# NazirNayal8/RbA

Measured on AMD Instinct MI355X. Metric: images/sec @1024x2048 Swin-B-1dl (RbA inference hot path), higher is better.
Workload: dtype f32 (f16x3 split-MFMA GEMMs, fp32 accumulate)

## Files before the change

### include/rba_hip.h

```cpp
#ifndef RBA_HIP_H
#define RBA_HIP_H

#include <stdint.h>

#ifdef __cplusplus
extern "C" {
#endif

int rba_hip_version(void);

int rba_set_concurrent_streams(int n);

int rba_reduce_f32(const float* mask, const float* cls_prob, float* rba, float* sem_seg, int32_t* argmax,
                   int Q, int K, int64_t HW, int score_mode, void* stream);

int rba_reduce_ws_f32(const float* mask, const float* cls_prob, float* rba, float* sem_seg, int32_t* argmax, int Q, int K,
                      int64_t HW, int score_mode, void* workspace, void* stream);

int rba_reduce_up4_f32(const float* mask_lowres, const float* cls_prob, float* rba, float* sem_seg,
                       int32_t* argmax, int Q, int K, int h, int w, int crop_h, int crop_w, int score_mode, void* stream);

int rba_resample_bilinear_f32(const float* in, const float* add, float* out, int C, int h, int w, int H, int W,
                              void* stream);

// ... 40 lines not shown
int64_t rba_group_norm_nhwc_workspace_bytes(int B, int P, int C, int G);
int rba_group_norm_nhwc_f32(const float* x, const float* gamma, const float* beta, float* y, float* workspace, int B, int P, int C,
                            int G, float eps, int relu, void* stream);
int rba_resample_bilinear_nhwc_f32(const float* in, const float* add, float* out, int C, int h, int w, int H, int W, void* stream);

int rba_add_layer_norm_f32(const float* x, const float* t, const float* t_bias, const float* gamma, const float* beta,
                           float* sum_out, float* y, int64_t rows, int C, float eps, void* stream);

int rba_merge_layer_norm_f32(const float* x, const float* gamma, const float* beta, float* y, int B, int H, int W, int Cin, float eps,
                             void* stream);

int rba_skinny_linear_f32(const float* x, const float* weight, const float* bias, float* out, int M, int N, int K,
                          int relu, void* stream);
int rba_skinny_linear_add_f32(const float* x, const float* x_add, int add_cols, const float* weight, const float* bias, float* out,
                              int M, int N, int K, int relu, int seg_n, void* stream);

int rba_split_weight_bf16x3(const float* weight, void* packed, int N, int K, void* stream);
int rba_split_linear_f32(const float* x, const void* weight_packed, const float* bias, float* out, int64_t M, int N, int K,
                         int act, void* stream);

int rba_split_weight_f16x2(const float* weight, void* packed, int N, int K, void* stream);
int rba_split_linear_f16x3_f32(const float* x, const void* weight_packed, const float* bias, float* out, int64_t M, int N, int K,
                               int act, void* stream);
int rba_split_linear_f16x3_res_f32(const float* x, const void* weight_packed, const float* bias, const float* residual, float* out,
                                   int64_t M, int N, int K, void* stream);

int rba_add_layer_norm_frag_f32(const float* x, const float* t, const float* t_bias, const float* gamma, const float* beta,
                                float* sum_out, void* y_frag, int64_t rows, int C, float eps, void* stream);
int rba_split_linear_f16x3_frag_f32(const void* x_frag, const void* weight_packed, const float* bias, const float* residual, float* out,
                                    int64_t M, int N, int K, int act, void* stream);
int rba_swin_window_attn_split_out_f32(const float* qkv, const float* qkv_bias, const float* bias_frag, void* out_frag, int B, int H, int W,
                                       int nH, int hd, int ws, int shift, void* stream);
int rba_swin_attn_block_supported(int C, int ws);
int64_t rba_swin_attn_block_weight_bytes(int C);
int rba_swin_attn_block_pack_f32(const float* qkv_weight, const float* proj_weight, void* image, int C, void* stream);
int rba_swin_attn_block_f32(float* x, float* y2, const float* norm1_weight, const float* norm1_bias, float eps1, const void* weight_image,
                            const float* qkv_bias, const float* bias_frag, const float* proj_bias, const float* norm2_weight,
                            const float* norm2_bias, float eps2, int B, int H, int W, int C, int ws, int shift, void* stream);
int rba_swin_attn_qkv_supported(int C, int ws);
int rba_swin_attn_qkv_split_out_f32(const float* x, void* out_frag, const float* norm1_weight, const float* norm1_bias, float eps1,
                                    const void* weight_image, const float* qkv_bias, const float* bias_frag, int B, int H, int W, int C, int ws,
                                    int shift, void* stream);
int rba_resample_bilinear_nhwc_split_out_f32(const float* in, const float* add, void* out_frag, int C, int h, int w, int H, int W,
                                             int64_t row0, void* stream);

int rba_resample_bilinear_nhwc_gn_f32(const float* in, const float* in_mr, const float* in_gamma, const float* in_beta, int in_relu,
                                      const float* add, const float* add_mr, const float* add_gamma, const float* add_beta, void* out,
                                      int split_out, int C, int G, int h, int w, int H, int W, int64_t row0, void* stream);
int rba_group_norm_nhwc_stats_f32(const float* x, float* mr, float* workspace, int B, int P, int C, int G, float eps, void* stream);
int rba_conv3x3_nhwc_f16x3_split_in_f32(const void* x_frag, const void* weight_packed, const float* bias, float* out, int B, int H, int W,
                                        int C, int N, void* stream);
int rba_swin_mlp_fused_f16x3_f32(const float* x, const void* w1_packed, const float* b1, const void* w2_packed, const float* b2,
                                 const float* residual, float* out, int64_t M, int C, int HID, void* stream);
int rba_swin_mlp_fused_ln_f16x3_f32(float* x, const float* norm_weight, const float* norm_bias, float eps, const void* w1_packed, const float* b1,
                                    const void* w2_packed, const float* b2, int64_t M, int C, int HID, void* stream);
int rba_split_linear_f16x3_gelu_split_out(const void* x, int x_is_split, const void* weight_packed, const float* bias, void* out_frag,
                                          int64_t M, int N, int K, void* stream);

int rba_split_linear_nchw_out_f32(const float* x, const void* weight_packed, const float* bias, float* out, int64_t M, int N,
                                  int K, int rows_per_image, void* stream);

int rba_split_linear_nchw_out_f16x3_f32(const float* x, const void* weight_packed, const float* bias, float* out, int64_t M, int N, int K,
                                        int rows_per_image, void* stream);

int rba_split_linear_nchw_out_gn_f16x3_f32(const float* x, const float* mr, const float* gamma, const float* beta, int G, int relu,
                                           const void* weight_packed, const float* bias, float* out, int64_t M, int N, int K,
                                           int rows_per_image, void* stream);

int rba_conv3x3_nhwc_f32(const float* x, const void* weight_packed, const float* bias, float* out, int B, int H, int W, int C,
                         int N, void* stream);

int rba_conv3x3_nhwc_f16x3_f32(const float* x, const void* weight_packed, const float* bias, float* out, int B, int H, int W, int C,
                               int N, void* stream);

int rba_split_linear_f16x3_gn_moments_f32(const float* x, const void* weight_packed, const float* bias, float* out, int64_t M, int N, int K,
                                          int rows_per_image, int G, float* moments, void* stream);
int rba_conv3x3_nhwc_f16x3_split_in_gn_moments_f32(const void* x_frag, const void* weight_packed, const float* bias, float* out, int B, int H,
                                                   int W, int C, int N, int G, float* moments, void* stream);
int rba_group_norm_nhwc_merge_f32(const float* moments, float* mr, int B, int G, int splits, float eps, void* stream);

int rba_patch_im2col_u8(const uint8_t* image, float* out, int h, int w, int Hp, int Wp, const float* mean, const float* std, void* stream);
int rba_patch_im2col_f32(const float* image, float* out, int h, int w, int Hp, int Wp, const float* mean, const float* std, void* stream);

int rba_gaussian_blur_f32(const float* in, float* out, int H, int W, int kernel_size, float sigma, void* stream);

int rba_quad_mean_f32(const float* v, float* out, int64_t rows, int S, void* stream);
int rba_softmax_drop_last_f32(const float* logits, float* prob, int64_t rows, int K1, void* stream);

int rba_threshold_u8(const float* score, uint8_t* out, int64_t n, float threshold, void* stream);
int rba_morph3x3_u8(const uint8_t* in, uint8_t* out, int H, int W, int dilate, void* stream);
int rba_ccl4_roots_i32(const uint8_t* mask, int32_t* roots, int H, int W, void* stream);

int rba_bn_relu_conv1x1_f32(const float* x, const float* scale, const float* shift, const float* weight, const float* bias, float* out,
                            int B, int C, int O, int64_t P, void* stream);
int rba_resample_bilinear_ac_f32(const float* x, float* out, int C, int h, int w, int H, int W, void* stream);

typedef struct {
  const float* x_add;
  const void* packed;
  const float* bias;
  float* out;
  int N;
  int ld_out;
  int act;
} rba_token_linear_problem;
int rba_token_linear_pack_f16x2(const float* weight, void* packed, int N, int K, void* stream);
int rba_token_linear_f32(const float* x, const float* x_add, const void* packed, const float* bias, const float* residual,
                         const float* ln_weight, const float* ln_bias, float ln_eps, float* out, int64_t M, int N, int K, int act,
                         void* stream);
int rba_token_linear_multi_f32(const float* x, const rba_token_linear_problem* problems, int n_problems, int64_t M, int K, void* stream);

#ifdef __cplusplus
}
#endif
#endif
```

### rba_amd/_lib.py

```python
import ctypes
import os

_HERE = os.path.dirname(os.path.abspath(__file__))
LIB_PATH = os.environ.get("RBA_HIP_LIB") or os.path.join(_HERE, "csrc", "librba_hip.so")
KNOBS_LIB_PATH = os.path.join(_HERE, "csrc", "librba_hip_knobs.so")

_c_f32p = ctypes.c_void_p
_i = ctypes.c_int
_i64 = ctypes.c_int64
_vp = ctypes.c_void_p

SIGNATURES = {
    "rba_hip_version": [],
    "rba_set_concurrent_streams": [_i],
    "rba_reduce_f32": [_vp, _vp, _vp, _vp, _vp, _i, _i, _i64, _i, _vp],
    "rba_reduce_ws_f32": [_vp, _vp, _vp, _vp, _vp, _i, _i, _i64, _i, _vp, _vp],
    "rba_reduce_up4_f32": [_vp, _vp, _vp, _vp, _vp, _i, _i, _i, _i, _i, _i, _i, _vp],
    "rba_resample_bilinear_f32": [_vp, _vp, _vp, _i, _i, _i, _i, _i, _vp],
    "rba_ms_deform_attn_fwd_f32": [_vp, _vp, _vp, _vp, _vp, _vp, _i, _i, _i, _i, _i, _i, _i, _vp],
    "rba_ms_deform_attn_fwd_f64": [_vp, _vp, _vp, _vp, _vp, _vp, _i, _i, _i, _i, _i, _i, _i, _vp],
    "rba_ms_deform_attn_bwd_f32": [_vp, _vp, _vp, _vp, _vp, _vp, _vp, _vp, _vp, _i, _i, _i, _i, _i, _i, _i, _vp],
    "rba_ms_deform_attn_bwd_f64": [_vp, _vp, _vp, _vp, _vp, _vp, _vp, _vp, _vp, _i, _i, _i, _i, _i, _i, _i, _vp],
    "rba_msda_prepare_f32": [_vp, _vp, _vp, _vp, _vp, _i64, _i, _i, _i, _vp],
    "rba_resample_bilinear_nhwc_gn_f32": [_vp, _vp, _vp, _vp, _i, _vp, _vp, _vp, _vp, _vp, _i, _i, _i, _i, _i, _i, _i, _i64, _vp],
    "rba_group_norm_nhwc_stats_f32": [_vp, _vp, _vp, _i, _i, _i, _i, ctypes.c_float, _vp],
    "rba_msda_fused_f32": [_vp, _vp, _vp, _vp, _vp, _vp, _i, _i, _i, _i, _i, _i, _i, _vp],
    "rba_masked_xattn_workspace_bytes": [_i, _i, _i, _i],
    "rba_masked_xattn_f32": [_vp, _vp, _vp, _vp, _vp, _vp, _i, _i, _i, _i, _i, _vp],
    "rba_mask_logits_f32": [_vp, _vp, _vp, _i, _i, _i, _i64, _vp],
    "rba_mask_logits_f16x3_f32": [_vp, _vp, _vp, _i, _i, _i, _i64, _vp],
    "rba_swin_window_attn_f32": [_vp, _vp, _vp, _vp, _vp, _i, _i, _i, _i, _i, _i, _i, _vp],
    "rba_swin_window_attn_split_out_f32": [_vp, _vp, _vp, _vp, _i, _i, _i, _i, _i, _i, _i, _vp],
    "rba_swin_bias_fragments_elems": [_i, _i],
    "rba_swin_attn_block_supported": [_i, _i],
    "rba_swin_attn_block_weight_bytes": [_i],
    "rba_swin_attn_qkv_supported": [_i, _i],
    "rba_swin_attn_qkv_split_out_f32": [_vp, _vp, _vp, _vp, ctypes.c_float, _vp, _vp, _vp, _i, _i, _i, _i, _i, _i, _vp],
    "rba_swin_attn_block_pack_f32": [_vp, _vp, _vp, _i, _vp],
    "rba_swin_attn_block_f32": [_vp, _vp, _vp, _vp, ctypes.c_float, _vp, _vp, _vp, _vp, _vp, _vp, ctypes.c_float, _i, _i, _i, _i, _i, _i, _vp],
    "rba_swin_bias_fragments_f32": [_vp, _vp, _i, _i, _vp],
    "rba_skinny_linear_f32": [_vp, _vp, _vp, _vp, _i, _i, _i, _i, _vp],
    "rba_skinny_linear_add_f32": [_vp, _vp, _i, _vp, _vp, _vp, _i, _i, _i, _i, _i, _vp],
    "rba_split_weight_bf16x3": [_vp, _vp, _i, _i, _vp],
    "rba_split_linear_f32": [_vp, _vp, _vp, _vp, _i64, _i, _i, _i, _vp],
    "rba_split_weight_f16x2": [_vp, _vp, _i, _i, _vp],
    "rba_split_linear_f16x3_f32": [_vp, _vp, _vp, _vp, _i64, _i, _i, _i, _vp],
    "rba_split_linear_f16x3_res_f32": [_vp, _vp, _vp, _vp, _vp, _i64, _i, _i, _vp],
    "rba_split_linear_f16x3_frag_f32": [_vp, _vp, _vp, _vp, _vp, _i64, _i, _i, _i, _vp],
    "rba_swin_mlp_fused_f16x3_f32": [_vp, _vp, _vp, _vp, _vp, _vp, _vp, _i64, _i, _i, _vp],
    "rba_swin_mlp_fused_ln_f16x3_f32": [_vp, _vp, _vp, ctypes.c_float, _vp, _vp, _vp, _vp, _i64, _i, _i, _vp],
    "rba_split_linear_f16x3_gelu_split_out": [_vp, _i, _vp, _vp, _vp, _i64, _i, _i, _vp],
    "rba_split_linear_nchw_out_f32": [_vp, _vp, _vp, _vp, _i64, _i, _i, _i, _vp],
    "rba_split_linear_nchw_out_f16x3_f32": [_vp, _vp, _vp, _vp, _i64, _i, _i, _i, _vp],
    "rba_split_linear_f16x3_gn_moments_f32": [_vp, _vp, _vp, _vp, _i64, _i, _i, _i, _i, _vp, _vp],
    "rba_conv3x3_nhwc_f16x3_split_in_gn_moments_f32": [_vp, _vp, _vp, _vp, _i, _i, _i, _i, _i, _i, _vp, _vp],
    "rba_group_norm_nhwc_merge_f32": [_vp, _vp, _i, _i, _i, ctypes.c_float, _vp],
    "rba_split_linear_nchw_out_gn_f16x3_f32": [_vp, _vp, _vp, _vp, _i, _i, _vp, _vp, _vp, _i64, _i, _i, _i, _vp],
    "rba_conv3x3_nhwc_f32": [_vp, _vp, _vp, _vp, _i, _i, _i, _i, _i, _vp],
    "rba_conv3x3_nhwc_f16x3_f32": [_vp, _vp, _vp, _vp, _i, _i, _i, _i, _i, _vp],
    "rba_conv3x3_nhwc_f16x3_split_in_f32": [_vp, _vp, _vp, _vp, _i, _i, _i, _i, _i, _vp],
    "rba_resample_bilinear_nhwc_split_out_f32": [_vp, _vp, _vp, _i, _i, _i, _i, _i, _i64, _vp],
    "rba_patch_im2col_u8": [_vp, _vp, _i, _i, _i, _i, _vp, _vp, _vp],
    "rba_patch_im2col_f32": [_vp, _vp, _i, _i, _i, _i, _vp, _vp, _vp],
    "rba_group_norm_nhwc_workspace_bytes": [_i, _i, _i, _i],
    "rba_group_norm_nhwc_f32": [_vp, _vp, _vp, _vp, _vp, _i, _i, _i, _i, ctypes.c_float, _i, _vp],
    "rba_resample_bilinear_nhwc_f32": [_vp, _vp, _vp, _i, _i, _i, _i, _i, _vp],
    "rba_bn_relu_conv1x1_f32": [_vp, _vp, _vp, _vp, _vp, _vp, _i, _i, _i, _i64, _vp],
    "rba_resample_bilinear_ac_f32": [_vp, _vp, _i, _i, _i, _i, _i, _vp],
    "rba_gaussian_blur_f32": [_vp, _vp, _i, _i, _i, ctypes.c_float, _vp],
    "rba_quad_mean_f32": [_vp, _vp, _i64, _i, _vp],
    "rba_softmax_drop_last_f32": [_vp, _vp, _i64, _i, _vp],
    "rba_threshold_u8": [_vp, _vp, _i64, ctypes.c_float, _vp],
    "rba_morph3x3_u8": [_vp, _vp, _i, _i, _i, _vp],
    "rba_ccl4_roots_i32": [_vp, _vp, _i, _i, _vp],
    "rba_add_layer_norm_f32": [_vp, _vp, _vp, _vp, _vp, _vp, _vp, _i64, _i, ctypes.c_float, _vp],
    "rba_add_layer_norm_frag_f32": [_vp, _vp, _vp, _vp, _vp, _vp, _vp, _i64, _i, ctypes.c_float, _vp],
    "rba_merge_layer_norm_f32": [_vp, _vp, _vp, _vp, _i, _i, _i, _i, ctypes.c_float, _vp],
    "rba_group_norm_workspace_bytes": [_i, _i, _i, _i],
    "rba_group_norm_f32": [_vp, _vp, _vp, _vp, _vp, _i, _i, _i, _i, ctypes.c_float, _i, _vp],
    "rba_token_linear_pack_f16x2": [_vp, _vp, _i, _i, _vp],
    "rba_token_linear_f32": [_vp, _vp, _vp, _vp, _vp, _vp, _vp, ctypes.c_float, _vp, _i64, _i, _i, _i, _vp],
    "rba_token_linear_multi_f32": [_vp, _vp, _i, _i64, _i, _vp],
}

class TokenLinearProblem(ctypes.Structure):
    _fields_ = [("x_add", ctypes.c_void_p), ("packed", ctypes.c_void_p), ("bias", ctypes.c_void_p), ("out", ctypes.c_void_p),
                ("N", ctypes.c_int), ("ld_out", ctypes.c_int), ("act", ctypes.c_int)]


EXPECTED_ABI = 191

_lib = None


class RbaHipError(RuntimeError):
    pass


def load():
    global _lib
    if _lib is not None:
        return _lib
    _lib = _open(LIB_PATH)
    return _lib


_handles = {}


def _open(path):
    if path in _handles:
        return _handles[path]
    import torch
    if not os.path.exists(path):
        raise RbaHipError(
            f"{path} not found: build it with `python -m rba_amd.csrc.build` (hipcc --offload-arch=gfx950; --knobs for the knobs build). "
            "rba_amd has no CPU or PyTorch fallback for its HIP kernels.")
    lib = ctypes.CDLL(path)
    for name, argtypes in SIGNATURES.items():
        try:
            fn = getattr(lib, name)
        except AttributeError as e:
            raise RbaHipError(f"{path} does not export {name}; rebuild it") from e
        fn.argtypes = argtypes
        fn.restype = ctypes.c_int64 if name.endswith(("_bytes", "_elems")) else ctypes.c_int
    abi = int(lib.rba_hip_version())
    if abi != EXPECTED_ABI:
        raise RbaHipError(f"{path} has ABI version {abi}, these bindings are written for {EXPECTED_ABI}; rebuild it "
                          "(python -m rba_amd.csrc.build)")
    _handles[path] = lib
    return lib


class use_library:

    def __init__(self, path):
        self.path = path

    def __enter__(self):
        global _lib
        self.prev = _lib
        _lib = _open(self.path)
        return _lib

    def __exit__(self, *exc):
        global _lib
# ... 26 lines not shown
```

### rba_amd/csrc/build.py

```python
import os
import subprocess
import sys
from concurrent.futures import ThreadPoolExecutor

HERE = os.path.dirname(os.path.abspath(__file__))
SOURCES = ["rba_reduce.hip", "resample.hip", "ms_deform_attn.hip", "ms_deform_attn_bwd.hip", "masked_xattn.hip", "mask_logits.hip",
           "swin_window_attn.hip", "swin_attn_block.hip", "group_norm.hip", "layer_norm.hip", "skinny_linear.hip", "split_linear.hip", "split_linear_dma.hip", "split_linear_gnf.hip", "gaussian_blur.hip", "open_panoptic.hip", "dense_hybrid.hip", "patch_embed.hip", "token_linear.hip", "decoder_small.hip"]
HEADERS = ["common.h", "knobs.h", "rba_reduce_kernels.h", "split_linear_dma.h", "split_linear_h3.h", "split_linear_h3q.h", "mlp_fused_h3.h", "swin_window_attn_h3.h", "swin_attn_block.h",
           os.path.join("..", "..", "include", "rba_hip.h")]
TUNE_SOURCES = [os.path.join("tune", "rba_reduce_tune.hip"), os.path.join("tune", "split_linear_tune.hip"), os.path.join("tune", "split_linear_ws.hip"), os.path.join("tune", "mlp_fused_h1.hip"), os.path.join("tune", "k5_timing.hip"), os.path.join("tune", "k5_wpe_ab.hip"), os.path.join("tune", "k5_wpe_plain.hip"), os.path.join("tune", "k5_persist.hip"), os.path.join("tune", "k7_timing.hip")] + [os.path.join("tune", f"gnf_form{f}_dbg{d}.hip") for f in (0, 1) for d in (0, 1)] + [os.path.join("tune", "gnf_form0_dbg1_unpacked.hip"), os.path.join("tune", "gnf_form1_dbg0_unpacked.hip")]
TUNE_LIB = os.path.join(HERE, "tune", "librba_tune.so")
LIB = os.path.join(HERE, "librba_hip.so")
KNOBS_LIB = os.path.join(HERE, "librba_hip_knobs.so")
KNOBS = ["-DRBA_TUNE_KNOBS"]
OBJ = os.path.join(HERE, "build")
HIPCC = os.environ.get("HIPCC", "/opt/rocm/bin/hipcc")
FLAGS = ["--offload-arch=gfx950", "-O3", "-std=c++17", "-fPIC", "-ffp-contract=fast", "-Wno-unused-result"]
NO_PACKED_FP32 = ["-Xclang", "-target-feature", "-Xclang", "-packed-fp32-ops"]
MFMA_SOURCES = ({"split_linear.hip", "split_linear_dma.hip", "mask_logits.hip", "masked_xattn.hip", "skinny_linear.hip"}
                if os.environ.get("RBA_NO_PACKED_FP32") == "1" else set())
UNPACKED_ALWAYS = {"split_linear_gnf.hip", "ms_deform_attn_bwd.hip"}
UNPACKED_SOURCES = MFMA_SOURCES | UNPACKED_ALWAYS


def _run(cmd):
    r = subprocess.run(cmd, cwd=HERE, stderr=subprocess.PIPE, text=True)
    err = "\n".join(ln for ln in r.stderr.splitlines() if "not a recognized feature for this target" not in ln)
    if err.strip():
        print(err, file=sys.stderr, flush=True)
    if r.returncode:
        raise subprocess.CalledProcessError(r.returncode, cmd)


def _stale(target, deps) -> bool:
    if not os.path.exists(target):
        return True
    t = os.path.getmtime(target)
    return any(os.path.getmtime(d) > t for d in deps)


def stale() -> bool:
    return _stale(LIB, [os.path.join(HERE, f) for f in SOURCES + HEADERS])


def build(force: bool = False, verbose: bool = True, knobs: bool = False) -> str:
    lib = KNOBS_LIB if knobs else LIB
    if not force and not _stale(lib, [os.path.join(HERE, f) for f in SOURCES + HEADERS]):
        return lib
    obj_dir = os.path.join(OBJ, "knobs") if knobs else OBJ
    os.makedirs(obj_dir, exist_ok=True)
    hdrs = [os.path.join(HERE, h) for h in HEADERS]

    def compile_one(src):
        s, o = os.path.join(HERE, src), os.path.join(obj_dir, src.replace(".hip", ".o"))
        if force or _stale(o, [s] + hdrs):
            cmd = [HIPCC] + FLAGS + (KNOBS if knobs else []) + (NO_PACKED_FP32 if src in UNPACKED_SOURCES else []) + ["-c", s, "-o", o]
            if verbose:
                print(" ".join(cmd), flush=True)
            _run(cmd)
        return o

    with ThreadPoolExecutor(max_workers=min(8, os.cpu_count() or 1)) as ex:
        objs = list(ex.map(compile_one, SOURCES))
    _link_and_gate(objs, lib, verbose)
    return lib


def _link_and_gate(objs, lib, verbose):
    tmp = lib + ".unscanned"
    cmd = [HIPCC, "--offload-arch=gfx950", "-shared", "-fPIC"] + objs + ["-o", tmp]
    if verbose:
        print(" ".join(cmd), flush=True)
    subprocess.run(cmd, check=True, cwd=HERE)
    try:
        from . import isa_hazards
    except ImportError:
        sys.path.insert(0, HERE)
        import isa_hazards
    try:
        r = isa_hazards.gate(tmp)
    except Exception:
        os.remove(tmp)
        raise
    if verbose:
        print(f"isa_hazards: {os.path.basename(lib)}: {r['code_objects']} code objects clean (rules D, T, P)", flush=True)
    os.replace(tmp, lib)


def build_knobs(force: bool = False, verbose: bool = True) -> str:
    return build(force=force, verbose=verbose, knobs=True)
# ... 29 lines not shown
```

### rba_amd/modeling/backbone/swin.py

```python
from types import SimpleNamespace

import torch
import torch.nn as nn
import torch.nn.functional as F

from ... import ops
from ...lru import derived
from ...registry import BACKBONE_REGISTRY


def relative_position_index(ws: int) -> torch.Tensor:
    ar = torch.arange(ws)
    gy, gx = torch.meshgrid(ar, ar, indexing="ij")
    gy, gx = gy.reshape(-1), gx.reshape(-1)
    dy = gy[:, None] - gy[None, :] + (ws - 1)
    dx = gx[:, None] - gx[None, :] + (ws - 1)
    return dy * (2 * ws - 1) + dx


class WindowAttention(nn.Module):
    def __init__(self, dim, window_size, num_heads):
        super().__init__()
        self.dim, self.window_size, self.num_heads = dim, window_size, num_heads
        self.relative_position_bias_table = nn.Parameter(torch.zeros((2 * window_size - 1) ** 2, num_heads))
# ... 61 lines not shown
            x = ops.linear(y, a.proj, residual=x)
            hidden = self.mlp.fc1.out_features
            y = ops.add_layer_norm(x, self.norm2.weight, self.norm2.bias, self.norm2.eps, frag=ops.linear_takes_split(M, hidden, C))[1]
            y = ops.linear(y, self.mlp.fc1, gelu=True, split_out=ops.linear_takes_split(M, C, hidden))
            return ops.linear(y, self.mlp.fc2, residual=x), None
        x, y = ops.add_layer_norm(x, self.norm1.weight, self.norm1.bias, self.norm1.eps, t, tb, inplace_sum=True,
                                  frag=ops.linear_takes_split(M, 3 * C, C))
        qkv = ops.linear(y, a.qkv)
        bias, bias_frag = a.gathered_bias()
        fused = ops.linear_residual_fused(M, C, C)
        y = ops.swin_window_attn(qkv, a.qkv.bias, bias, H, W, self.num_heads, self.window_size, self.shift_size, bias_frag=bias_frag,
                                 split_out=fused and bias_frag is not None and ops.linear_takes_split(M, C, C) and
                                 ops.swin_window_attn_split_ok(C // self.num_heads, self.window_size))
        if fused:
            x = ops.linear(y, a.proj, residual=x)
            hidden = self.mlp.fc1.out_features
            if ops.mlp_fused_ok(M, C, hidden):
                y = ops.add_layer_norm(x, self.norm2.weight, self.norm2.bias, self.norm2.eps)[1]
                return ops.mlp_fused(y, self.mlp.fc1, self.mlp.fc2, x), None
            y = ops.add_layer_norm(x, self.norm2.weight, self.norm2.bias, self.norm2.eps, frag=ops.linear_takes_split(M, hidden, C))[1]
            y = ops.linear(y, self.mlp.fc1, gelu=True, split_out=ops.linear_takes_split(M, C, hidden))
            return ops.linear(y, self.mlp.fc2, residual=x), None
        t = ops.linear(y, a.proj, use_bias=False)
        x, y = ops.add_layer_norm(x, self.norm2.weight, self.norm2.bias, self.norm2.eps, t, a.proj.bias, inplace_sum=True)
        y = ops.linear(y, self.mlp.fc1, gelu=True)
        return x, (ops.linear(y, self.mlp.fc2, use_bias=False), self.mlp.fc2.bias)


class PatchMerging(nn.Module):
    def __init__(self, dim):
        super().__init__()
        self.reduction = nn.Linear(4 * dim, 2 * dim, bias=False)
        self.norm = nn.LayerNorm(4 * dim)

    def forward(self, x, H, W):
        x = ops.merge_layer_norm(x.contiguous(), H, W, self.norm.weight, self.norm.bias, self.norm.eps)
        return ops.linear(x, self.reduction)


class BasicLayer(nn.Module):
    def __init__(self, dim, depth, num_heads, window_size, mlp_ratio, downsample):
        super().__init__()
        self.blocks = nn.ModuleList(
            SwinTransformerBlock(dim, num_heads, window_size, 0 if i % 2 == 0 else window_size // 2, mlp_ratio)
            for i in range(depth))
        self.downsample = PatchMerging(dim) if downsample else None


class PatchEmbed(nn.Module):
    def __init__(self, patch_size, in_chans, embed_dim):
        super().__init__()
        self.patch_size = patch_size
        self.proj = nn.Conv2d(in_chans, embed_dim, kernel_size=patch_size, stride=patch_size)
        self.norm = nn.LayerNorm(embed_dim)

    def forward(self, x):
        ps = self.patch_size
        _, _, H, W = x.shape
        if W % ps or H % ps:
            x = F.pad(x, (0, (ps - W % ps) % ps, 0, (ps - H % ps) % ps))
        B, Cin, H, W = x.shape
        Wh, Ww = H // ps, W // ps
        cols = x.reshape(B, Cin, Wh, ps, Ww, ps).permute(0, 2, 4, 1, 3, 5).reshape(B, Wh * Ww, Cin * ps * ps).contiguous()
        x = ops.linear(cols, self._linear_view())
        return ops.add_layer_norm(x, self.norm.weight, self.norm.bias, self.norm.eps)[1], Wh, Ww

    def _linear_view(self):
        w, b = self.proj.weight, self.proj.bias
        return derived(self, "linear_view", (w, b), lambda: SimpleNamespace(weight=w.detach().reshape(w.shape[0], -1), bias=b))

    def fused_ok(self):
        w = self.proj.weight
        return self.patch_size == 4 and w.shape[1] == 3 and w.is_cuda and w.dtype == torch.float32 and ops.SPLIT_MODE == "f16x3"

    def forward_images(self, images, mean, std, Hp, Wp):
        w = self.proj.weight

        def build():
            w64 = torch.zeros((w.shape[0], 64), dtype=torch.float32, device=w.device)
            w64[:, :48] = w.detach().reshape(w.shape[0], 48)
            return ops.split_weight(w64, mode="f16x3")

        planes = derived(self, "planes64", (w,), build)
        cols = torch.stack([ops.patch_im2col(im, mean, std, Hp, Wp) for im in images]) if len(images) > 1 \
            else ops.patch_im2col(images[0], mean, std, Hp, Wp)[None]
        x = ops.split_linear(cols, planes, self.proj.bias, out_features=w.shape[0])
        return ops.add_layer_norm(x, self.norm.weight, self.norm.bias, self.norm.eps)[1], Hp // 4, Wp // 4


@BACKBONE_REGISTRY.register()
class D2SwinTransformer(nn.Module):

    def __init__(self, arch):
        super().__init__()
        E, depths = arch["embed_dim"], arch["depths"]
        self.patch_embed = PatchEmbed(arch["patch_size"], 3, E)
        self.layers = nn.ModuleList(
            BasicLayer(E * 2 ** i, depths[i], arch["num_heads"][i], arch["window_size"], arch["mlp_ratio"],
                       downsample=i < len(depths) - 1) for i in range(len(depths)))
        self.num_features = [E * 2 ** i for i in range(len(depths))]
        for i, c in enumerate(self.num_features):
            self.add_module(f"norm{i}", nn.LayerNorm(c))

    @property
    def size_divisibility(self):
        return 32

    def forward_images(self, images, mean, std, Hp, Wp):
        return self._stages(*self.patch_embed.forward_images(images, mean, std, Hp, Wp))

    def forward(self, x):
        if x.dim() != 4:
            raise ValueError(f"SwinTransformer takes an input of shape (N, C, H, W). Got {tuple(x.shape)} instead!")
        return self._stages(*self.patch_embed(x))

    def _stages(self, x, Wh, Ww):
        outs = {}
        for i, layer in enumerate(self.layers):
            pending = None
            for blk in layer.blocks:
                x, pending = blk(x, Wh, Ww, pending)
            norm = getattr(self, f"norm{i}")
            t, tb = pending if pending is not None else (None, None)
            x, y = ops.add_layer_norm(x, norm.weight, norm.bias, norm.eps, t, tb, inplace_sum=True)
            outs[f"res{i + 2}"] = y.view(-1, Wh, Ww, self.num_features[i]).permute(0, 3, 1, 2)
            if layer.downsample is not None:
                x = layer.downsample(x, Wh, Ww)
                Wh, Ww = (Wh + 1) // 2, (Ww + 1) // 2
        return outs
```

### rba_amd/ops.py

```python
import contextlib
import ctypes
import threading
import functools
import math
import os

import torch

from . import _lib
from ._lib import RbaHipError
from .lru import derived


def _stream():
    return torch.cuda.current_stream().cuda_stream


def _cuda_tensors(args):
    for a in args:
        if isinstance(a, torch.Tensor):
            if a.is_cuda:
                yield a
        elif isinstance(a, (list, tuple)):
            yield from _cuda_tensors(a)
# ... 993 lines not shown

@_hip_op
def token_linear(x, lin, x_add=None, use_bias=True, relu=False, residual=None, norm=None):
    lib = _lib.load()
    _chk(x, "x")
    N, K = lin.weight.shape
    if x.shape[-1] != K or not token_linear_ok(N, K):
        raise RbaHipError("token_linear: x [..., K] with K % 32 == 0, N <= 256 and the f16x3 mode (see token_linear_ok)")
    M = x.numel() // K
    if x_add is not None:
        _chk(x_add, "x_add")
        if tuple(x_add.shape) != tuple(x.shape):
            raise RbaHipError("x_add must have x's shape")
    bias = lin.bias if use_bias else None
    if bias is not None:
        _chk(bias, "bias", dim=1)
    out = torch.empty(tuple(x.shape[:-1]) + (N,), dtype=torch.float32, device=x.device)
    if (residual is None) != (norm is None):
        raise RbaHipError("token_linear: residual and norm come together")
    if norm is not None:
        _chk(residual, "residual")
        if tuple(residual.shape) != tuple(out.shape) or N % 16 or relu or norm.weight.numel() != N:
            raise RbaHipError("token_linear(norm=...): residual [..., N], N % 16 == 0, no activation")
        _lib.check(lib.rba_token_linear_f32(_p(x), _p(x_add), _p(_token_planes(lin)), _p(bias), _p(residual), _p(norm.weight), _p(norm.bias),
                                            float(norm.eps), _p(out), M, N, K, 0, _stream()), "rba_token_linear_f32")
        return out
    _lib.check(lib.rba_token_linear_f32(_p(x), _p(x_add), _p(_token_planes(lin)), _p(bias), None, None, None, 0.0, _p(out), M, N, K,
                                        2 if relu else 0, _stream()), "rba_token_linear_f32")
    return out


@_hip_op
def token_linear_multi(x, specs):
    lib = _lib.load()
    _chk(x, "x")
    K = x.shape[-1]
    M = x.numel() // K if K else 0
    if not 1 <= len(specs) <= 3:
        raise RbaHipError("token_linear_multi: one to three problems")
    arr = (_lib.TokenLinearProblem * len(specs))()
    outs, keep = [], []
    for i, (lin, x_add, out, col0, relu) in enumerate(specs):
        N, K_ = lin.weight.shape
        if K_ != K or not token_linear_ok(N, K) or N % 4:
            raise RbaHipError("token_linear_multi: weights [N <= 256, N % 4 == 0, K] with x's K % 32 == 0 (see token_linear_ok)")
        if x_add is not None:
            _chk(x_add, "x_add")
            if tuple(x_add.shape) != tuple(x.shape):
                raise RbaHipError("x_add must have x's shape")
        if out is None:
            out, col0 = torch.empty(tuple(x.shape[:-1]) + (N,), dtype=torch.float32, device=x.device), 0
        else:
            _chk(out, "out")
            if tuple(out.shape[:-1]) != tuple(x.shape[:-1]) or col0 % 4 or col0 + N > out.shape[-1] or out.shape[-1] % 4:
                raise RbaHipError("token_linear_multi: out [..., ld] with ld % 4 == 0 and a column slice col0 % 4 == 0 inside it")
        if lin.bias is not None:
            _chk(lin.bias, "bias", dim=1)
        planes = _token_planes(lin)
        keep.append(planes)
        arr[i] = _lib.TokenLinearProblem(_p(x_add) or None, _p(planes), _p(lin.bias) or None, out.data_ptr() + 4 * col0, N, out.shape[-1], 2 if relu else 0)
        outs.append(out)
    _lib.check(lib.rba_token_linear_multi_f32(_p(x), ctypes.byref(arr), len(specs), M, K, _stream()), "rba_token_linear_multi_f32")
    return outs


@_hip_op
def patch_im2col(image, mean, std, Hp, Wp):
    import ctypes
    lib = _lib.load()
    if image.dtype not in (torch.uint8, torch.float32):
        raise RbaHipError("image must be uint8 or float32")
    _chk(image, "image", dtype=image.dtype, dim=3)
    if image.shape[0] != 3 or Hp % 4 or Wp % 4 or Hp < image.shape[1] or Wp < image.shape[2] or len(mean) != 3 or len(std) != 3:
        raise RbaHipError("patch_im2col needs a [3,h,w] image and Hp >= h, Wp >= w multiples of 4")
    h, w = int(image.shape[1]), int(image.shape[2])
    out = torch.empty(((Hp // 4) * (Wp // 4), 64), dtype=torch.float32, device=image.device)
    m = (ctypes.c_float * 3)(*[float(v) for v in mean])
    sd = (ctypes.c_float * 3)(*[float(v) for v in std])
    fn, name = ((lib.rba_patch_im2col_u8, "rba_patch_im2col_u8") if image.dtype == torch.uint8 else (lib.rba_patch_im2col_f32, "rba_patch_im2col_f32"))
    _lib.check(fn(_p(image), _p(out), h, w, int(Hp), int(Wp), ctypes.addressof(m), ctypes.addressof(sd), _stream()), name)
    return out


@_hip_op
def group_norm_nhwc(x, num_groups, weight, bias, eps=1e-5, relu=False):
    lib = _lib.load()
    _chk(x, "x")
    _chk(weight, "weight", dim=1)
    _chk(bias, "bias", dim=1)
    if x.dim() not in (3, 4):
        raise RbaHipError("x must be [B,P,C] or [B,H,W,C]")
    B, C = x.shape[0], x.shape[-1]
    P = x.numel() // (B * C) if B * C else 0
    if C % num_groups or weight.numel() != C or bias.numel() != C or (C // num_groups) % 4 or C > 1024 or 256 % (C // 4):
        raise RbaHipError("group_norm_nhwc needs C % G == 0, (C/G) % 4 == 0, C <= 1024 and 256 % (C/4) == 0")
    nbytes = lib.rba_group_norm_nhwc_workspace_bytes(B, P, C, num_groups)
    ws = torch.empty(max(nbytes // 4, 1), dtype=torch.float32, device=x.device)
    y = torch.empty_like(x)
    _lib.check(lib.rba_group_norm_nhwc_f32(_p(x), _p(weight), _p(bias), _p(y), _p(ws), B, P, C, num_groups, float(eps),
                                           int(bool(relu)), _stream()), "rba_group_norm_nhwc_f32")
    return y


@_hip_op
def resample_bilinear_nhwc(x, size, add=None, split_into=None, image=0):
    lib = _lib.load()
    _chk(x, "x", dim=3)
    h, w, C = x.shape
    H, W = int(size[0]), int(size[1])
    if C % 4:
        raise RbaHipError("resample_bilinear_nhwc needs C % 4 == 0")
    if add is not None:
        _chk(add, "add")
        if tuple(add.shape) != (H, W, C):
            raise RbaHipError("add must have the output's shape")
    if split_into is not None:
        if (not isinstance(split_into, SplitActivations) or len(split_into.shape) != 4 or tuple(split_into.shape[1:]) != (H, W, C) or C % 32
                or not 0 <= image < split_into.shape[0]):
            raise RbaHipError("split_into must be SplitActivations of shape [B, H, W, C] (C % 32 == 0) with 0 <= image < B")
        _lib.check(lib.rba_resample_bilinear_nhwc_split_out_f32(_p(x), _p(add), _p(split_into.data), C, h, w, H, W, image * H * W, _stream()),
                   "rba_resample_bilinear_nhwc_split_out_f32")
        return split_into
    out = torch.empty((H, W, C), dtype=torch.float32, device=x.device)
    _lib.check(lib.rba_resample_bilinear_nhwc_f32(_p(x), _p(add), _p(out), C, h, w, H, W, _stream()),
               "rba_resample_bilinear_nhwc_f32")
    return out


def _gn_nhwc_ok(C, num_groups):
    return C % num_groups == 0 and (C // num_groups) % 4 == 0 and C <= 1024 and 256 % (C // 4) == 0


@_hip_op
def group_norm_nhwc_stats(x, num_groups, eps=1e-5):
    lib = _lib.load()
    _chk(x, "x")
    if x.dim() not in (3, 4):
        raise RbaHipError("x must be [B,P,C] or [B,H,W,C]")
    B, C = x.shape[0], x.shape[-1]
    P = x.numel() // (B * C) if B * C else 0
    if not _gn_nhwc_ok(C, num_groups):
        raise RbaHipError("group_norm_nhwc_stats needs C % G == 0, (C/G) % 4 == 0, C <= 1024 and 256 % (C/4) == 0")
    nbytes = lib.rba_group_norm_nhwc_workspace_bytes(B, P, C, num_groups)
    ws = torch.empty(max(nbytes // 4, 1), dtype=torch.float32, device=x.device)
    mr = torch.empty((B, num_groups, 2), dtype=torch.float32, device=x.device)
    _lib.check(lib.rba_group_norm_nhwc_stats_f32(_p(x), _p(mr), _p(ws), B, P, C, num_groups, float(eps), _stream()), "rba_group_norm_nhwc_stats_f32")
    return mr


@_hip_op
def resample_bilinear_nhwc_gn(x, size, add, num_groups, x_norm=None, add_norm=None, split_into=None, image=0):
    lib = _lib.load()
    _chk(x, "x", dim=3)
    _chk(add, "add", dim=3)
    h, w, C = x.shape
    H, W = int(size[0]), int(size[1])
    if tuple(add.shape) != (H, W, C) or not _gn_nhwc_ok(C, num_groups):
        raise RbaHipError("resample_bilinear_nhwc_gn: add must be [H, W, C]; C % G == 0, (C/G) % 4 == 0")

    def unpack(n, with_relu):
        if n is None:
            return 0, 0, 0, 0
        mr, wgt, b = n[0], n[1], n[2]
        _chk(mr, "mr")
        _chk(wgt, "weight", dim=1)
        _chk(b, "bias", dim=1)
# ... 113 lines not shown
```

Before: 147.3.

## Fuse patch im2col, f16x3 patch-embed GEMM and LayerNorm into one kernel

Adds a single HIP kernel that normalizes image pixels, forms 4x4 patches in registers, runs the 64->128 patch projection with split-f16 MFMA, adds bias and applies LayerNorm before writing tokens. It replaces the im2col kernel, the split_linear GEMM and the separate add_layer_norm, removing two intermediate global-memory round trips and two launches. It is used by default for E=128, patch size 4 and f16x3 mode, and can be turned off with RBA_PATCH_FUSED=0. Risks include lower occupancy from the weights held in LDS and registers, and small numerical differences in the LayerNorm reduction.

```diff
diff --git a/include/rba_hip.h b/include/rba_hip.h
--- a/include/rba_hip.h
+++ b/include/rba_hip.h
@@ -146,6 +146,11 @@
 int rba_patch_im2col_u8(const uint8_t* image, float* out, int h, int w, int Hp, int Wp, const float* mean, const float* std, void* stream);
 int rba_patch_im2col_f32(const float* image, float* out, int h, int w, int Hp, int Wp, const float* mean, const float* std, void* stream);
 
+int rba_patch_embed_ln_u8(const uint8_t* image, const void* weight_packed, const float* bias, const float* gamma, const float* beta, float* out,
+                          int h, int w, int Hp, int Wp, int E, const float* mean, const float* std, float eps, void* stream);
+int rba_patch_embed_ln_f32(const float* image, const void* weight_packed, const float* bias, const float* gamma, const float* beta, float* out,
+                           int h, int w, int Hp, int Wp, int E, const float* mean, const float* std, float eps, void* stream);
+
 int rba_gaussian_blur_f32(const float* in, float* out, int H, int W, int kernel_size, float sigma, void* stream);
 
 int rba_quad_mean_f32(const float* v, float* out, int64_t rows, int S, void* stream);
diff --git a/rba_amd/_lib.py b/rba_amd/_lib.py
--- a/rba_amd/_lib.py
+++ b/rba_amd/_lib.py
@@ -62,6 +62,8 @@
     "rba_resample_bilinear_nhwc_split_out_f32": [_vp, _vp, _vp, _i, _i, _i, _i, _i, _i64, _vp],
     "rba_patch_im2col_u8": [_vp, _vp, _i, _i, _i, _i, _vp, _vp, _vp],
     "rba_patch_im2col_f32": [_vp, _vp, _i, _i, _i, _i, _vp, _vp, _vp],
+    "rba_patch_embed_ln_u8": [_vp, _vp, _vp, _vp, _vp, _vp, _i, _i, _i, _i, _i, _vp, _vp, ctypes.c_float, _vp],
+    "rba_patch_embed_ln_f32": [_vp, _vp, _vp, _vp, _vp, _vp, _i, _i, _i, _i, _i, _vp, _vp, ctypes.c_float, _vp],
     "rba_group_norm_nhwc_workspace_bytes": [_i, _i, _i, _i],
     "rba_group_norm_nhwc_f32": [_vp, _vp, _vp, _vp, _vp, _i, _i, _i, _i, ctypes.c_float, _i, _vp],
     "rba_resample_bilinear_nhwc_f32": [_vp, _vp, _vp, _i, _i, _i, _i, _i, _vp],
diff --git a/rba_amd/csrc/build.py b/rba_amd/csrc/build.py
--- a/rba_amd/csrc/build.py
+++ b/rba_amd/csrc/build.py
@@ -5,7 +5,7 @@
 
 HERE = os.path.dirname(os.path.abspath(__file__))
 SOURCES = ["rba_reduce.hip", "resample.hip", "ms_deform_attn.hip", "ms_deform_attn_bwd.hip", "masked_xattn.hip", "mask_logits.hip",
-           "swin_window_attn.hip", "swin_attn_block.hip", "group_norm.hip", "layer_norm.hip", "skinny_linear.hip", "split_linear.hip", "split_linear_dma.hip", "split_linear_gnf.hip", "gaussian_blur.hip", "open_panoptic.hip", "dense_hybrid.hip", "patch_embed.hip", "token_linear.hip", "decoder_small.hip"]
+           "swin_window_attn.hip", "swin_attn_block.hip", "group_norm.hip", "layer_norm.hip", "skinny_linear.hip", "split_linear.hip", "split_linear_dma.hip", "split_linear_gnf.hip", "gaussian_blur.hip", "open_panoptic.hip", "dense_hybrid.hip", "patch_embed.hip", "patch_embed_ln.hip", "token_linear.hip", "decoder_small.hip"]
 HEADERS = ["common.h", "knobs.h", "rba_reduce_kernels.h", "split_linear_dma.h", "split_linear_h3.h", "split_linear_h3q.h", "mlp_fused_h3.h", "swin_window_attn_h3.h", "swin_attn_block.h",
            os.path.join("..", "..", "include", "rba_hip.h")]
 TUNE_SOURCES = [os.path.join("tune", "rba_reduce_tune.hip"), os.path.join("tune", "split_linear_tune.hip"), os.path.join("tune", "split_linear_ws.hip"), os.path.join("tune", "mlp_fused_h1.hip"), os.path.join("tune", "k5_timing.hip"), os.path.join("tune", "k5_wpe_ab.hip"), os.path.join("tune", "k5_wpe_plain.hip"), os.path.join("tune", "k5_persist.hip"), os.path.join("tune", "k7_timing.hip")] + [os.path.join("tune", f"gnf_form{f}_dbg{d}.hip") for f in (0, 1) for d in (0, 1)] + [os.path.join("tune", "gnf_form0_dbg1_unpacked.hip"), os.path.join("tune", "gnf_form1_dbg0_unpacked.hip")]
diff --git a/rba_amd/csrc/patch_embed_ln.hip b/rba_amd/csrc/patch_embed_ln.hip
--- /dev/null
+++ b/rba_amd/csrc/patch_embed_ln.hip
@@ -0,0 +1,173 @@
+#define RBA_H3_HELPERS_ONLY
+#include "split_linear_h3.h"
+#include "../../include/rba_hip.h"
+
+namespace {
+
+struct PatchNorm {
+  float m0, m1, m2, s0, s1, s2;
+};
+
+template <typename T, bool FAST>
+__device__ __forceinline__ f32x4 patch_segment(const T* row, int x0, int w, float mean, float sd) {
+  f32x4 v = {0.f, 0.f, 0.f, 0.f};
+  if (!row) return v;
+  if constexpr (FAST && sizeof(T) == 4) {
+    if (x0 < w) {
+      const f32x4 p = *reinterpret_cast<const f32x4*>(row + x0);
+#pragma unroll
+      for (int kx = 0; kx < 4; ++kx) v[kx] = ((float)p[kx] - mean) / sd;
+    }
+  } else if constexpr (FAST) {
+    if (x0 < w) {
+      const uint32_t p = *reinterpret_cast<const uint32_t*>(row + x0);
+      v[0] = ((float)(p & 0xffu) - mean) / sd;
+      v[1] = ((float)((p >> 8) & 0xffu) - mean) / sd;
+      v[2] = ((float)((p >> 16) & 0xffu) - mean) / sd;
+      v[3] = ((float)(p >> 24) - mean) / sd;
+    }
+  } else {
+#pragma unroll
+    for (int kx = 0; kx < 4; ++kx)
+      if (x0 + kx < w) v[kx] = ((float)row[x0 + kx] - mean) / sd;
+  }
+  return v;
+}
+
+template <typename T, bool FAST>
+__global__ __launch_bounds__(256, 2) void patch_embed_ln_kernel(const T* __restrict__ img, const u32x4_t* __restrict__ Wp, const float* __restrict__ bias,
+                                                                const float* __restrict__ gamma, const float* __restrict__ beta,
+                                                                float* __restrict__ out, int h, int w, int Wt, int tokens, PatchNorm pn, float eps) {
+  constexpr int E = 128, CT = 4, SUBW = 4 * E;
+  __shared__ __attribute__((aligned(16))) u32x4_t wl[4 * SUBW];
+  const int tid = threadIdx.x, lane = tid & 63;
+  const int wave = __builtin_amdgcn_readfirstlane(tid >> 6);
+  const int l31 = lane & 31, lh = lane >> 5;
+  const int m0 = blockIdx.x * 128;
+
+  u32x4_t wr[8];
+#pragma unroll
+  for (int q = 0; q < 8; ++q) wr[q] = Wp[tid + 256 * q];
+  const int token = m0 + 32 * wave + l31;
+  const bool tvalid = token < tokens;
+  const int ty = (tvalid ? token : 0) / Wt, tx = (tvalid ? token : 0) - ty * Wt;
+  const int x0 = 4 * tx;
+  f32x4 xs[2][4];
+#pragma unroll
+  for (int b = 0; b < 2; ++b) {
+    const int c = 2 * b + lh;
+    const float mean = c == 0 ? pn.m0 : (c == 1 ? pn.m1 : pn.m2), sd = c == 0 ? pn.s0 : (c == 1 ? pn.s1 : pn.s2);
+#pragma unroll
+    for (int ky = 0; ky < 4; ++ky) {
+      const int y = 4 * ty + ky;
+      const T* row = (tvalid && c < 3 && y < h) ? img + ((int64_t)c * h + y) * w : nullptr;
+      xs[b][ky] = patch_segment<T, FAST>(row, x0, w, mean, sd);
+    }
+  }
+#pragma unroll
+  for (int q = 0; q < 8; ++q) wl[tid + 256 * q] = wr[q];
+  __syncthreads();
+
+  f32x16_t accm[CT], accl[CT];
+#pragma unroll
+  for (int j = 0; j < CT; ++j)
+#pragma unroll
+    for (int r = 0; r < 16; ++r) accm[j][r] = accl[j][r] = 0.f;
+  const int fb = l31 * 2 + (lh ^ ((l31 >> 3) & 1));
+#pragma unroll
+  for (int b = 0; b < 2; ++b) {
+#pragma unroll
+    for (int g = 0; g < 2; ++g) {
+      f16x8_t ah, al;
+      split_h3(xs[b][2 * g], xs[b][2 * g + 1], ah, al);
+      const u32x4_t* im = wl + (2 * b + g) * SUBW + fb;
+      f16x8_t bh[CT], bl[CT];
+#pragma unroll
+      for (int j = 0; j < CT; ++j) {
+        bh[j] = __builtin_bit_cast(f16x8_t, im[64 * j]);
+        bl[j] = __builtin_bit_cast(f16x8_t, im[2 * E + 64 * j]);
+      }
+#pragma unroll
+      for (int j = 0; j < CT; ++j) accm[j] = __builtin_amdgcn_mfma_f32_32x32x16_f16(ah, bh[j], accm[j], 0, 0, 0);
+#pragma unroll
+      for (int j = 0; j < CT; ++j) accl[j] = __builtin_amdgcn_mfma_f32_32x32x16_f16(ah, bl[j], accl[j], 0, 0, 0);
+#pragma unroll
+      for (int j = 0; j < CT; ++j) accl[j] = __builtin_amdgcn_mfma_f32_32x32x16_f16(al, bh[j], accl[j], 0, 0, 0);
+    }
+  }
+
+  float ga[CT], be[CT];
+#pragma unroll
+  for (int j = 0; j < CT; ++j) {
+    const float bv = bias[32 * j + l31];
+    ga[j] = gamma[32 * j + l31];
+    be[j] = beta[32 * j + l31];
+#pragma unroll
+    for (int r = 0; r < 16; r += 2) {
+      f32x2 y = (f32x2){accl[j][r], accl[j][r + 1]} * 0.00048828125f + (f32x2){accm[j][r], accm[j][r + 1]};
+      y = y + bv;
+      accm[j][r] = y.x;
+      accm[j][r + 1] = y.y;
+    }
+  }
+  const int rbase = m0 + 32 * wave + 4 * lh;
+  const bool full = m0 + 128 <= tokens;
+  float* dst = out + (int64_t)rbase * E + l31;
+#pragma unroll
+  for (int r = 0; r < 16; ++r) {
+    float sum = (accm[0][r] + accm[1][r]) + (accm[2][r] + accm[3][r]);
+#pragma unroll
+    for (int o = 16; o > 0; o >>= 1) sum += __shfl_xor(sum, o, RBA_WAVE);
+    const float mean = sum / (float)E;
+    float d[CT];
+#pragma unroll
+    for (int j = 0; j < CT; ++j) d[j] = accm[j][r] - mean;
+    float sq = (d[0] * d[0] + d[1] * d[1]) + (d[2] * d[2] + d[3] * d[3]);
+#pragma unroll
+    for (int o = 16; o > 0; o >>= 1) sq += __shfl_xor(sq, o, RBA_WAVE);
+    const float rstd = 1.0f / sqrtf(sq / (float)E + eps);
+    const int ro = 8 * (r >> 2) + (r & 3);
+    if (full || rbase + ro < tokens) {
+#pragma unroll
+      for (int j = 0; j < CT; ++j) dst[(int64_t)ro * E + 32 * j] = d[j] * rstd * ga[j] + be[j];
+    }
+  }
+}
+
+template <typename T>
+int launch_patch_embed_ln(const T* img, const void* wp, const float* bias, const float* gamma, const float* beta, float* out, int h, int w, int Hp,
+                          int Wp, const float* mean, const float* sd, float eps, hipStream_t st) {
+  const int Wt = Wp / 4;
+  const int64_t tokens = (int64_t)(Hp / 4) * Wt;
+  const PatchNorm pn{mean[0], mean[1], mean[2], sd[0], sd[1], sd[2]};
+  const dim3 grid((unsigned)((tokens + 127) / 128));
+  const u32x4_t* wpk = reinterpret_cast<const u32x4_t*>(wp);
+  const bool fast = (w & 3) == 0 && ((uintptr_t)img & (4 * sizeof(T) - 1)) == 0;
+  if (fast)
+    hipLaunchKernelGGL((patch_embed_ln_kernel<T, true>), grid, dim3(256), 0, st, img, wpk, bias, gamma, beta, out, h, w, Wt, (int)tokens, pn, eps);
+  else
+    hipLaunchKernelGGL((patch_embed_ln_kernel<T, false>), grid, dim3(256), 0, st, img, wpk, bias, gamma, beta, out, h, w, Wt, (int)tokens, pn, eps);
+  return rba_launch_status();
+}
+
+}
+
+#define RBA_PATCH_EMBED_LN_ARGS                                                                                                              \
+  RBA_CHECK_ARG(image && weight_packed && bias && gamma && beta && out && mean && std && E == 128);                                          \
+  RBA_CHECK_ARG(h >= 1 && w >= 1 && Hp >= h && Wp >= w && (Hp % 4) == 0 && (Wp % 4) == 0 && (int64_t)Hp * Wp < (int64_t)1 << 31);            \
+  RBA_CHECK_ARG((((uintptr_t)weight_packed | (uintptr_t)out) & 15) == 0 && (((uintptr_t)bias | (uintptr_t)gamma | (uintptr_t)beta) & 3) == 0)
+
+extern "C" int rba_patch_embed_ln_u8(const uint8_t* image, const void* weight_packed, const float* bias, const float* gamma, const float* beta,
+                                     float* out, int h, int w, int Hp, int Wp, int E, const float* mean, const float* std, float eps, void* stream) {
+  RBA_PATCH_EMBED_LN_ARGS;
+  rba_begin();
+  return launch_patch_embed_ln<uint8_t>(image, weight_packed, bias, gamma, beta, out, h, w, Hp, Wp, mean, std, eps, (hipStream_t)stream);
+}
+
+extern "C" int rba_patch_embed_ln_f32(const float* image, const void* weight_packed, const float* bias, const float* gamma, const float* beta,
+                                      float* out, int h, int w, int Hp, int Wp, int E, const float* mean, const float* std, float eps, void* stream) {
+  RBA_PATCH_EMBED_LN_ARGS;
+  RBA_CHECK_ARG(((uintptr_t)image & 3) == 0);
+  rba_begin();
+  return launch_patch_embed_ln<float>(image, weight_packed, bias, gamma, beta, out, h, w, Hp, Wp, mean, std, eps, (hipStream_t)stream);
+}
diff --git a/rba_amd/modeling/backbone/swin.py b/rba_amd/modeling/backbone/swin.py
--- a/rba_amd/modeling/backbone/swin.py
+++ b/rba_amd/modeling/backbone/swin.py
@@ -167,6 +167,12 @@
             return ops.split_weight(w64, mode="f16x3")
 
         planes = derived(self, "planes64", (w,), build)
+        if ops.patch_embed_fused_ok(w.shape[0], self.patch_size, w.shape[1], isinstance(self.norm, nn.LayerNorm)):
+            T = (Hp // 4) * (Wp // 4)
+            x = torch.empty((len(images), T, w.shape[0]), dtype=torch.float32, device=w.device)
+            for i, im in enumerate(images):
+                ops.patch_embed_ln(im, mean, std, Hp, Wp, planes, self.proj.bias, self.norm.weight, self.norm.bias, self.norm.eps, out=x[i])
+            return x, Hp // 4, Wp // 4
         cols = torch.stack([ops.patch_im2col(im, mean, std, Hp, Wp) for im in images]) if len(images) > 1 \
             else ops.patch_im2col(images[0], mean, std, Hp, Wp)[None]
         x = ops.split_linear(cols, planes, self.proj.bias, out_features=w.shape[0])
diff --git a/rba_amd/ops.py b/rba_amd/ops.py
--- a/rba_amd/ops.py
+++ b/rba_amd/ops.py
@@ -1099,6 +1099,43 @@
     return out
 
 
+PATCH_FUSED = os.environ.get("RBA_PATCH_FUSED", "1") != "0"
+
+
+def patch_embed_fused_ok(embed_dim, patch_size=4, in_chans=3, patch_norm=True):
+    return PATCH_FUSED and embed_dim == 128 and patch_size == 4 and in_chans == 3 and bool(patch_norm) and _split_mode() == "f16x3"
+
+
+@_hip_op
+def patch_embed_ln(image, mean, std, Hp, Wp, planes, bias, gamma, beta, eps=1e-5, out=None):
+    lib = _lib.load()
+    if image.dtype not in (torch.uint8, torch.float32):
+        raise RbaHipError("image must be uint8 or float32")
+    _chk(image, "image", dtype=image.dtype, dim=3)
+    if image.shape[0] != 3 or Hp % 4 or Wp % 4 or Hp < image.shape[1] or Wp < image.shape[2] or len(mean) != 3 or len(std) != 3:
+        raise RbaHipError("patch_embed_ln needs a [3,h,w] image and Hp >= h, Wp >= w multiples of 4")
+    _chk(planes, "planes", dtype=torch.float16)
+    for t, name in ((bias, "bias"), (gamma, "gamma"), (beta, "beta")):
+        _chk(t, name, dim=1)
+    E = int(gamma.numel())
+    if E != 128 or bias.numel() != E or beta.numel() != E or tuple(planes.shape) != (1, 4, 2, 128, 2, 8):
+        raise RbaHipError("patch_embed_ln needs E = 128 and the f16x3 planes of the [128, 64] weight (check patch_embed_fused_ok first)")
+    h, w = int(image.shape[1]), int(image.shape[2])
+    tokens = (Hp // 4) * (Wp // 4)
+    if out is None:
+        out = torch.empty((tokens, E), dtype=torch.float32, device=image.device)
+    else:
+        _chk(out, "out", dim=2)
+        if tuple(out.shape) != (tokens, E):
+            raise RbaHipError(f"out must be [{tokens}, {E}]")
+    m = (ctypes.c_float * 3)(*[float(v) for v in mean])
+    sd = (ctypes.c_float * 3)(*[float(v) for v in std])
+    fn, name = ((lib.rba_patch_embed_ln_u8, "rba_patch_embed_ln_u8") if image.dtype == torch.uint8 else (lib.rba_patch_embed_ln_f32, "rba_patch_embed_ln_f32"))
+    _lib.check(fn(_p(image), _p(planes), _p(bias), _p(gamma), _p(beta), _p(out), h, w, int(Hp), int(Wp), E, ctypes.addressof(m), ctypes.addressof(sd),
+                  float(eps), _stream()), name)
+    return out
+
+
 @_hip_op
 def group_norm_nhwc(x, num_groups, weight, bias, eps=1e-5, relu=False):
     lib = _lib.load()
```

New measurement: 148.1 (median of 6 runs). Within noise of the previous version (+0.6%).
